# VITA-Group/UVC

Hardware: AMD Instinct MI355X
Metric: images/sec UVC Stage-1 step, DeiT-Tiny budget=0.5 (higher is better)
Workload: dtype bf16; 1 GPU; deit_tiny_patch16_224 Stage-1 UVC-train step, budget 0.5, per-GPU batch 512, 224x224x3 synthetic, soft distillation alpha 0.1, block gating on; global_batch=512, parallelism=dp1

## Files before the change

### include/uvc_kernels.h

```cpp
#ifndef UVC_KERNELS_H
#define UVC_KERNELS_H
#include <stdint.h>
#ifdef __cplusplus
extern "C" {
#endif

enum { UVC_F32 = 0, UVC_BF16 = 1 };

enum {
  UVC_EPI_NONE = 0,
  UVC_EPI_BIAS = 1,
  UVC_EPI_BIAS_GELU = 2,
  UVC_EPI_BIAS_RESID = 3,
  UVC_EPI_BIAS_RESID_GATE = 4,
  UVC_EPI_DGELU = 5,
  UVC_EPI_BIAS_GELU_OUT = 6,
  UVC_EPI_BIAS_GELU_GRAD = 7,
  UVC_EPI_MUL_AUX = 8,
  UVC_EPI_BIAS_GELU_GRAD_Q8 = 9,
  UVC_EPI_MUL_AUX_Q8 = 10
};
#define UVC_Q8_LO (-0.13f)
#define UVC_Q8_STEP (1.26f / 255.0f)

// ... 70 lines not shown

typedef struct uvc_attn_tok_args {
  const void* qkv;
  void* o;
  const void* dout;
  void* dqkv;
  int32_t B, N, H, head_dim, ntok, dtype;
  float scale;
  const int32_t* head_keep;
} uvc_attn_tok_args;
int uvc_attention_tok_fwd(const uvc_attn_tok_args* args, void* stream);
int uvc_attention_tok_bwd(const uvc_attn_tok_args* args, void* stream);

int uvc_copy_row_groups(const void* src, void* dst, int64_t groups, int64_t group_bytes, int64_t src_group_stride, int64_t dst_group_stride,
                        void* stream);

typedef struct uvc_ln_args {
  const void* x;
  const float* gamma; const float* beta;
  void* y; float* mean; float* rstd;
  const void* dy;
  void* dx;
  const void* add1; const float* a1;
  const void* add2; const float* a2;
  float* partial;
  float* dgamma; float* dbeta;
  float* dots;
  float eps, beta_acc;
  int32_t rows, D, rows_per_group, dtype, y_is_f32, dy_is_f32;
  int64_t group_stride;
// ... 102 lines not shown
```

### uvc_amd/_lib.py

```python
from __future__ import annotations

import ctypes as C
import os

import torch

_HERE = os.path.dirname(os.path.abspath(__file__))
LIB_PATH = os.path.join(_HERE, "libuvc_hip.so")


class UvcHipError(RuntimeError):
    pass


class uvc_dims(C.Structure):
    _fields_ = [("L", C.c_int32), ("H", C.c_int32), ("hd", C.c_int32), ("D", C.c_int32), ("F", C.c_int32)]


class uvc_hyper(C.Structure):
    _fields_ = [(n, C.c_float) for n in ("budget", "slr", "rlr", "glr", "ylr", "plr", "zlr", "sl2wd", "z_grad_clip",
                                         "gating_weight", "eps")] + \
               [(n, C.c_int32) for n in ("gating_interval", "use_gumbel", "enable_block_gating")]


# ... 146 lines not shown
    "uvc_resource": [C.POINTER(uvc_state), uvc_dims, uvc_hyper, VP, C.c_int32, VP, VP],
    "uvc_write_masks": [VP, VP, VP, uvc_dims, VP, VP, VP, VP, VP, VP],
    "uvc_gemm_nt": [C.POINTER(uvc_gemm_nt_args), VP],
    "uvc_gemm_nt_ln_supported": [I32, I32, I32, I32, I32],
    "uvc_gemm_nt_q8_supported": [I32, I32, I32, I32],
    "uvc_gemm_tn": [C.POINTER(uvc_gemm_tn_args), VP],
    "uvc_gemm_tn_workspace_bytes": [I32, I32, I32, C.POINTER(I64), C.POINTER(I32)],
    "uvc_attention_fwd": [C.POINTER(uvc_attn_args), VP],
    "uvc_attention_bwd": [C.POINTER(uvc_attn_args), VP],
    "uvc_attention_bwd_vdim": [C.POINTER(uvc_attn_args), VP],
    "uvc_qkv_attention_supported": [I32, I32, I32, I32, I32],
    "uvc_qkv_attention_fwd": [C.POINTER(uvc_qkv_attn_args), VP],
    "uvc_attention_tok_fwd": [C.POINTER(uvc_attn_tok_args), VP],
    "uvc_attention_tok_bwd": [C.POINTER(uvc_attn_tok_args), VP],
    "uvc_copy_row_groups": [VP, VP, I64, I64, I64, I64, VP],
    "uvc_layernorm_fwd": [C.POINTER(uvc_ln_args), VP],
    "uvc_layernorm_bwd": [C.POINTER(uvc_ln_args), VP],
    "uvc_layernorm_bwd_blocks": [I32],
    "uvc_layernorm_bwd_nblocks": [I32],
    "uvc_layernorm_bwd_reduce_batch": [C.POINTER(uvc_ln_reduce_item), I32, I32, F32, VP],
    "uvc_gemm_lnbwd_supported": [I32, I32, I32, I32],
    "uvc_gemm_lnbwd_nblocks": [I32],
    "uvc_gemm_nt_lnbwd": [C.POINTER(uvc_gemm_lnbwd_args), VP],
    "uvc_distill_loss": [C.POINTER(uvc_loss_args), VP],
    "uvc_grad_sqnorm": [VP, I64, VP, VP, I32, VP],
    "uvc_adamw_step": [C.POINTER(uvc_adamw_args), VP],
    "uvc_scale_by_clip": [VP, I64, VP, F32, VP],
    "uvc_patchify": [VP, VP, I32, I32, I32, I32, I32, VP],
    "uvc_assemble_tokens": [VP, VP, VP, VP, VP, VP, I32, I32, I32, I32, I32, VP],
    "uvc_assemble_tokens_bwd": [VP, VP, VP, VP, VP, VP, VP, VP, I32, I32, I32, I32, I32, I32, I32, F32, VP],
# ... 93 lines not shown
```

### uvc_amd/csrc/gemm.hip

```cpp
#include <type_traits>
#include "common.h"
#include "../../include/uvc_kernels.h"

template <typename T> struct Mma;
template <> struct Mma<bf16_t> {
  static constexpr int CH = 8;
  static constexpr int KSTEP = 32;
  typedef bf16x8 Frag;
  static __device__ __forceinline__ f32x4 mma(const Frag& a, const Frag& b, f32x4 c) {
    return __builtin_amdgcn_mfma_f32_16x16x32_bf16(a, b, c, 0, 0, 0);
  }
};
template <> struct Mma<float> {
  static constexpr int CH = 4;
  static constexpr int KSTEP = 16;
  typedef f32x4 Frag;
  static __device__ __forceinline__ f32x4 mma(const Frag& a, const Frag& b, f32x4 c) {
#pragma unroll
    for (int j = 0; j < 4; ++j) c = __builtin_amdgcn_mfma_f32_16x16x4f32(a[j], b[j], c, 0, 0, 0);
    return c;
  }
};

template <typename TS, typename T> struct ChunkLoad;
// ... 851 lines not shown
    E = En;
    if (next < ntiles) lstore(par ? sA0 : sA1);
    __syncthreads();
    par ^= 1;
  }
}

static bool wsn_ok(const NtArgs& a, int epi, bool a_f32) {
  return !a_f32 && a.N == 192 && (a.K == 768 || a.K == 576 || a.K == 512 || a.K == 256) && a.ldb == a.K && a.lda % 8 == 0 && a.ldc % 4 == 0 && a.ldr % 4 == 0 && a.M >= 4096 &&
         (epi == UVC_EPI_NONE || epi == UVC_EPI_BIAS || epi == UVC_EPI_BIAS_RESID || epi == UVC_EPI_BIAS_RESID_GATE);
}
template <int EPI, int KT, bool LN, int NST, bool RLOW> __global__ void k_gemm_wsn16_dma(NtArgs g);
template <int EPI, int KT, bool LN, int NST, bool RLOW>
static int launch_wsn16_dma(const NtArgs& a, hipStream_t st) {
  constexpr int NX_ = RLOW ? 7 : 13;
  constexpr int NA_ = (16 * (KT * 4 + 2) + 63) / 64, NI_ = NA_ + NX_ + (EPI == UVC_EPI_BIAS_RESID_GATE ? NX_ : 0);
  const int sh = NST * NI_ * 1024 + (LN ? 2 * 16 * 12 * 8 + 3 * 192 * 4 : 0);
  UVC_MAX_LDS(sh, k_gemm_wsn16_dma<EPI, KT, LN, NST, RLOW>);
  const int ntiles = ceil_div(a.M, 16);
  k_gemm_wsn16_dma<EPI, KT, LN, NST, RLOW><<<ntiles < 256 ? ntiles : 256, 768, sh, st>>>(a);
  UVC_CHECK_LAUNCH();
  return UVC_OK;
}
static bool wsn16_dma_ok(const NtArgs& a) {
  return a.M >= 16 && a.lda == a.K && a.ldr == 192 && a.ldc % 4 == 0 && (((uintptr_t)a.R | (uintptr_t)a.R2 | (uintptr_t)a.A) & 15) == 0;
}
template <typename TC, int KT>
static int launch_wsn16_kt(const NtArgs& a, int epi, hipStream_t st) {
  if constexpr (KT == 24 || KT == 16 || KT == 8) {
    constexpr bool RLOW = sizeof(TC) == 2;
    const bool ok = (!a.no_dma || a.ln_out) && wsn16_dma_ok(a) && (a.ln_out || a.M % 16 == 0);
// ... 50 lines not shown
    case 512: return launch_wsn_kt<TC, 16>(a, epi, st);
    default: return launch_wsn_kt<TC, 8>(a, epi, st);
  }
}

template <typename TA, typename T, typename TC>
static int launch_nt_epi(const NtArgs& a, int epi, hipStream_t st) {
  const int grid = ceil_div(ceil_div(a.M, NT_BM), 8) * 8 * ceil_div(a.N, NT_BN);
#define NT_CASE(E) case E: k_gemm_nt<TA, T, TC, E><<<grid, 256, 0, st>>>(a); break;
  switch (epi) {
    NT_CASE(UVC_EPI_NONE) NT_CASE(UVC_EPI_BIAS) NT_CASE(UVC_EPI_BIAS_GELU) NT_CASE(UVC_EPI_BIAS_RESID)
    NT_CASE(UVC_EPI_BIAS_RESID_GATE) NT_CASE(UVC_EPI_DGELU) NT_CASE(UVC_EPI_BIAS_GELU_OUT) NT_CASE(UVC_EPI_BIAS_GELU_GRAD) NT_CASE(UVC_EPI_MUL_AUX)
    default: return uvc_set_error_msg(UVC_ERR_ARG, "uvc_gemm_nt: unknown epilogue");
  }
#undef NT_CASE
  UVC_CHECK_LAUNCH();
  return UVC_OK;
}

int launch_nt256_f32(const NtArgs& a, int epi, hipStream_t st);
int launch_nt256_bf16(const NtArgs& a, int epi, hipStream_t st);
bool nt256_takes(const NtArgs& a, bool a_f32, bool any_size);
int launch_nt8p_f32(const NtArgs& a, int epi, int ri, hipStream_t st);
int launch_nt8p_bf16(const NtArgs& a, int epi, int ri, hipStream_t st);
bool nt8p_takes(const NtArgs& a, bool a_f32);
bool row384_fwd_ok(const NtArgs& a, int epi);
int launch_row384_fwd(const NtArgs& a, int epi, hipStream_t st);
static bool row384_fwd_fits(int64_t M, int64_t K) { return (M + 128) * K * 2 < (1ll << 31); }

extern "C" int uvc_gemm_nt_ln_supported(int32_t M, int32_t N, int32_t K, int32_t dtype, int32_t epilogue) {
// ... 49 lines not shown
      return uvc_set_error_msg(UVC_ERR_UNSUPPORTED, "uvc_gemm_nt: ln_out is not available for this problem (uvc_gemm_nt_ln_supported)");
    if (p->M % 16 != 0 && (p->C == (const void*)p->R || p->C == (const void*)p->R2))
      return uvc_set_error_msg(UVC_ERR_ARG, "uvc_gemm_nt: with ln_out and M % 16 != 0 the last row tile is computed twice: C must not alias R / R2");
    if (p->K == 192) return p->c_is_f32 ? launch_wsn16_dma<UVC_EPI_BIAS_RESID, 6, true, 7, false>(a, st) : launch_wsn16_dma<UVC_EPI_BIAS_RESID, 6, true, 7, true>(a, st);
    return p->c_is_f32 ? launch_wsn<float>(a, e, st) : launch_wsn<bf16_t>(a, e, st);
  }
  if (p->dtype == UVC_F32) {
    if (!p->a_is_f32 || !p->c_is_f32) return uvc_set_error_msg(UVC_ERR_ARG, "uvc_gemm_nt: float32 mode needs float32 A and C");
    return launch_nt_epi<float, float, float>(a, e, st);
  }
  if (p->dtype != UVC_BF16) return uvc_set_error_msg(UVC_ERR_ARG, "uvc_gemm_nt: dtype must be UVC_F32 or UVC_BF16");
  {
    if (!p->force_generic && !p->a_is_f32 && e == UVC_EPI_BIAS_RESID && p->K == 192 && p->N == 192 && a.ldb == 192 &&
        p->M >= 4096 && p->M % 16 == 0 && p->alpha == 1.0f && !p->alpha_ptr && wsn16_dma_ok(a))
      return p->c_is_f32 ? launch_wsn16_dma<UVC_EPI_BIAS_RESID, 6, false, 7, false>(a, st) : launch_wsn16_dma<UVC_EPI_BIAS_RESID, 6, false, 7, true>(a, st);
  }
  const bool ws = !generic && ws_ok(a, p->c_is_f32 ? 4 : 8);
  if (q8 && !ws) return uvc_set_error_msg(UVC_ERR_UNSUPPORTED, "uvc_gemm_nt: the one-byte GELU' epilogues exist in the K = 192 streaming kernel only");
  if (!generic && ws384_ok(a, e, p->c_is_f32 ? 4 : 8, p->a_is_f32 != 0)) {
    if (!p->c_is_f32 && a.N % 128 == 0 && a.N >= 512 && p->force_generic != 5) return launch_ws384<bf16_t, 8>(a, e, st);
    return p->c_is_f32 ? launch_ws384<float>(a, e, st) : launch_ws384<bf16_t>(a, e, st);
  }
  if (!generic && wsn_ok(a, e, p->a_is_f32 != 0))
    return p->c_is_f32 ? launch_wsn<float>(a, e, st) : launch_wsn<bf16_t>(a, e, st);
  if ((p->force_generic >> 8) == 1) {
    if (!nt8p_takes(a, p->a_is_f32 != 0)) return uvc_set_error_msg(UVC_ERR_UNSUPPORTED, "uvc_gemm_nt: shape not taken by the 8-phase kernel");
    return p->c_is_f32 ? launch_nt8p_f32(a, e, p->force_generic & 255, st) : launch_nt8p_bf16(a, e, p->force_generic & 255, st);
  }
  const bool few_tiles_wide = !p->c_is_f32 && a.N % 256 == 0 && nt8p_takes(a, p->a_is_f32 != 0);
  if (!generic && !a.no_dma && !(p->force_generic == 3 && few_tiles_wide && a.N < 1792) &&
      nt256_takes(a, p->a_is_f32 != 0, p->force_generic == 3 || p->force_generic == 4))
    return p->c_is_f32 ? launch_nt256_f32(a, e, st) : launch_nt256_bf16(a, e, st);
  if (!generic && !a.no_dma && few_tiles_wide && (a.M >= 2048 || p->force_generic == 3))
    return launch_nt8p_bf16(a, e, 0, st);
  if (p->a_is_f32) {
    if ((p->lda % 8) != 0) return uvc_set_error_msg(UVC_ERR_ARG, "uvc_gemm_nt: lda");
    if (ws) return p->c_is_f32 ? launch_ws<float, float>(a, e, st) : launch_ws<float, bf16_t>(a, e, st);
    return p->c_is_f32 ? launch_nt_epi<float, bf16_t, float>(a, e, st) : launch_nt_epi<float, bf16_t, bf16_t>(a, e, st);
  }
  if (ws) return p->c_is_f32 ? launch_ws<bf16_t, float>(a, e, st) : launch_ws<bf16_t, bf16_t>(a, e, st);
  return p->c_is_f32 ? launch_nt_epi<bf16_t, bf16_t, float>(a, e, st) : launch_nt_epi<bf16_t, bf16_t, bf16_t>(a, e, st);
}

template <typename T> struct Raw4L;
template <> struct Raw4L<float> {
  typedef f32x4 V;
  static __device__ __forceinline__ V ld(const float* p) { return *reinterpret_cast<const f32x4*>(p); }
  static __device__ __forceinline__ V zero() { return f32x4{0.f, 0.f, 0.f, 0.f}; }
  static __device__ __forceinline__ f32x4 cvt(const V& r) { return r; }
};
template <> struct Raw4L<bf16_t> {
  typedef u32x2 V;
  static __device__ __forceinline__ V ld(const bf16_t* p) { return *reinterpret_cast<const u32x2*>(p); }
  static __device__ __forceinline__ V zero() { return u32x2{0u, 0u}; }
// ... 377 lines not shown
    for (int q = 0; q < NWV; ++q) t += sRed[2 * q + tid];
    P[2 * D + tid] = t;
  }
}
#undef TIE4

template <int EPI, int KT, bool LN, int NST, bool RLOW>
__global__ __launch_bounds__(768) void k_gemm_wsn16_dma(NtArgs g) {
  typedef bf16_t T;
  typedef Mma<T> MM;
  constexpr int K = KT * 32, D = 192, NWV = 12;
  constexpr int ROWB = K * 2 + 32, SA = ROWB / 16;
  constexpr int NA = (16 * SA + 63) / 64;
  constexpr int RSZ = RLOW ? 2 : 4, RSL = D * RSZ / 16;
  constexpr int XS = RSL + 2, XB = XS * 16, NX = (16 * XS + 63) / 64;
  constexpr bool GATE = EPI == UVC_EPI_BIAS_RESID_GATE;
  constexpr int I_R = NA, I_R2 = I_R + NX, NI = I_R2 + (GATE ? NX : 0);
  constexpr int STAGE = NI * 1024;
  constexpr int NPW = (NI + NWV - 1) / NWV;
  constexpr int LN_BYTES = LN ? 2 * 16 * NWV * 8 + 3 * D * 4 : 0;
  static_assert(NST >= 3 && NPW <= 5 && NST * STAGE + LN_BYTES <= 160 * 1024, "ring does not fit");
  extern __shared__ __attribute__((aligned(16))) char smem[];
  const int tid = threadIdx.x, lane = tid & 63, gq = lane >> 4, li = lane & 15;
  const int w = __builtin_amdgcn_readfirstlane(tid >> 6);
  const T* __restrict__ W = reinterpret_cast<const T*>(g.B);
  char* __restrict__ C = reinterpret_cast<char*>(g.C);
  const int ntiles = (g.M + 15) / 16;
  const int n = w * 16 + gq * 4;
  float* const sRed = reinterpret_cast<float*>(smem + NST * STAGE);
  float* const sGB = sRed + 2 * 16 * NWV * 2;
  if (LN) {
    if (tid < D) { sGB[tid] = g.ln_gamma[tid]; sGB[D + tid] = g.ln_beta[tid]; sGB[2 * D + tid] = g.bias[tid]; }
  }
  const unsigned gaddr = lds_addr(sGB) + (unsigned)n * 4u;
  const unsigned redr = lds_addr(sRed) + (unsigned)(li * NWV * 8);
  typename MM::Frag bf[KT];
#pragma unroll
  for (int ks = 0; ks < KT; ++ks)
    bf[ks] = __builtin_bit_cast(typename MM::Frag, *reinterpret_cast<const u32x4*>(W + (size_t)(w * 16 + li) * K + (ks * 4 + gq) * 8));
  float alpha = g.alpha;
  if (g.alpha_ptr) alpha *= *g.alpha_ptr;
  float d0 = 0.f, d1 = 1.f;
  if (GATE) { d0 = g.dptr[0]; d1 = g.dptr[1]; }
  f32x4 bias4 = {0.f, 0.f, 0.f, 0.f};
  if (!LN) bias4 = *reinterpret_cast<const f32x4*>(g.bias + n);

  const char* rb[NPW]; unsigned rstride[NPW], rdst[NPW], loff[NPW];
#pragma unroll
  for (int q = 0; q < NPW; ++q) {
    int I = q * NWV + w;
    if (I >= NI) I = w;
    const int sl = (I - (I < I_R ? 0 : I < I_R2 ? I_R : I_R2)) * 64 + lane;
    rdst[q] = (unsigned)I * 1024u;
    if (I < I_R) {
      const int row = sl / SA, c = sl % SA;
      rb[q] = reinterpret_cast<const char*>(g.A); rstride[q] = K * 2u;
      loff[q] = row < 16 ? (unsigned)(row * K * 2 + (c < K / 8 ? c : 0) * 16) : 0u;
    } else {
      const int row = sl / XS, c = sl % XS;
      rb[q] = reinterpret_cast<const char*>(I < I_R2 ? g.R : g.R2); rstride[q] = (unsigned)(D * RSZ);
      loff[q] = row < 16 ? (unsigned)(row * D * RSZ + (c < RSL ? c : 0) * 16) : 0u;
    }
  }
  auto issue = [&](int tile, int st) {
    const int t = tile < ntiles ? tile : ntiles - 1;
    const unsigned r0 = (unsigned)min(t * 16, g.M - 16);
#pragma unroll
    for (int q = 0; q < NPW; ++q) {
      const char* src = rb[q] + ((unsigned long long)r0 * (unsigned long long)rstride[q] + (unsigned long long)loff[q]);
      char* dst = smem + st * STAGE + rdst[q];
      __builtin_amdgcn_global_load_lds((const void __attribute__((address_space(1)))*)src, (void __attribute__((address_space(3)))*)dst, 16, 0, 0);
    }
  };
  const unsigned s0 = lds_addr(smem);
  const unsigned fragoff = (unsigned)(li * ROWB + gq * 16), roff = (unsigned)(I_R * 1024 + li * XB + n * RSZ);

  int tile = blockIdx.x;
#pragma unroll
  for (int q = 0; q < NST - 1; ++q) issue(tile + q * gridDim.x, q);
// ... 64 lines not shown
    if (LN && have_prev) { ln_first(); ln_issue(std::integral_constant<int, 32>{}); }
    GROUP(1, fb, fa)
    if (LN && have_prev) { ln_acc(); ln_issue(std::integral_constant<int, 64>{}); }
    GROUP(2, fa, fb)
    if (LN && have_prev) {
      ln_acc();
      if constexpr (KT / 2 > 3) { lgr = ds_read128<0>(gaddr); lbr = ds_read128<D * 4>(gaddr); }
      else { lgr = ds_read128<0>(gaddr); lbr = ds_read128<D * 4>(gaddr); wait_lgkm<0>(); ln_finish(); }
    }
    GROUP(3, fb, fa)
    if (LN && have_prev && KT / 2 > 3) ln_finish();
    GROUP(4, fa, fb) GROUP(5, fb, fa)
    GROUP(6, fa, fb) GROUP(7, fb, fa) GROUP(8, fa, fb) GROUP(9, fb, fa) GROUP(10, fa, fb) GROUP(11, fb, fa)
#undef GROUP
#undef RD2
    typename Resid<typename std::conditional<RLOW, bf16_t, float>::type>::Raw4 rr, rr2;
    if constexpr (RLOW) {
      asm volatile("ds_read_b64 %0, %1" : "=v"(rr) : "v"(sb + roff));
      rr2 = rr;
      if (GATE) asm volatile("ds_read_b64 %0, %1 offset:%2" : "=v"(rr2) : "v"(sb + roff), "n"(NX * 1024));
    } else {
      rr = ds_read128<0>(sb + roff); rr2 = rr;
      if (GATE) rr2 = ds_read128<NX * 1024>(sb + roff);
    }
    typedef Resid<typename std::conditional<RLOW, bf16_t, float>::type> RS;
    if constexpr (!LN) {
      wait_vm<(NST - 2) * NPW>();
      wait_lgkm<0>();
      asm volatile("" : "+v"(rr), "+v"(rr2));
      __builtin_amdgcn_s_barrier();
      const f32x4 r = RS::f4(rr), r2 = RS::f4(rr2);
      float o[4];
#pragma unroll
      for (int e = 0; e < 4; ++e) {
        o[e] = epi_scale_bias(c0[e], alpha, bias4[e]);
        o[e] += r[e];
        if (GATE) o[e] = epi_gate_mix(o[e], r2[e], d0, d1);
      }
      char* cp = C + ((size_t)(min(tile * 16, g.M - 16) + li) * g.ldc + n) * RSZ;
      if constexpr (RLOW) { u32x2 q; q[0] = pack_bf16x2(o[0], o[1]); q[1] = pack_bf16x2(o[2], o[3]); *reinterpret_cast<u32x2*>(cp) = q; }
      else *reinterpret_cast<f32x4*>(cp) = f32x4{o[0], o[1], o[2], o[3]};
    } else {
      u32x4 bq = ds_read128<2 * D * 4>(gaddr);
      wait_lgkm<0>();
      asm volatile("" : "+v"(rr), "+v"(rr2), "+v"(bq));
      const f32x4 r = RS::f4(rr), r2 = RS::f4(rr2), bv = __builtin_bit_cast(f32x4, bq);
      float o[4];
#pragma unroll
      for (int e = 0; e < 4; ++e) {
        o[e] = epi_scale_bias(c0[e], alpha, bv[e]);
        o[e] += r[e];
// ... 1584 lines not shown
```

### uvc_amd/csrc/token_tail.hip

```cpp
#include "common.h"
#include "../../include/uvc_kernels.h"

namespace {

constexpr int HD = 64, NTH = 256, MAXN = 256, MAXT = 2;

template <typename T> struct Row;
template <> struct Row<bf16_t> {
  static constexpr int WORDS = 33;
  static __device__ __forceinline__ void put8(uint32_t* row, int c, const bf16_t* src) {
    const u32x4 v = *reinterpret_cast<const u32x4*>(src);
#pragma unroll
    for (int e = 0; e < 4; ++e) row[c * 4 + e] = v[e];
  }
  static __device__ __forceinline__ float get(const uint32_t* row, int d) {
    const uint32_t w = row[d >> 1];
    return __uint_as_float((d & 1) ? (w & 0xffff0000u) : (w << 16));
  }
  static __device__ __forceinline__ float dot(const uint32_t* row, const float* q) {
    float s = 0.f;
#pragma unroll 8
    for (int i = 0; i < 32; ++i) {
      const uint32_t w = row[i];
      s = __builtin_fmaf(__uint_as_float(w << 16), q[2 * i], s);
// ... 205 lines not shown
  const dim3 grid(p->H, p->B);
  if (bwd) k_attn_tok_bwd<T><<<grid, NTH, sh, st>>>(a);
  else k_attn_tok_fwd<T><<<grid, NTH, sh, st>>>(a);
  UVC_CHECK_LAUNCH();
  return UVC_OK;
}

__global__ __launch_bounds__(256) void k_copy_row_groups(const char* __restrict__ src, char* __restrict__ dst, int64_t pieces, int ppg,
                                                         int64_t sgs, int64_t dgs) {
  const int64_t i = (int64_t)blockIdx.x * 256 + threadIdx.x;
  if (i >= pieces) return;
  const int64_t gi = i / ppg, r = i % ppg;
  *reinterpret_cast<u32x4*>(dst + gi * dgs + r * 16) = *reinterpret_cast<const u32x4*>(src + gi * sgs + r * 16);
}

}

extern "C" int uvc_attention_tok_fwd(const uvc_attn_tok_args* p, void* stream) {
  if (int e = tok_check(p, false)) return e;
  return p->dtype == UVC_F32 ? tok_launch<float>(p, false, (hipStream_t)stream) : tok_launch<bf16_t>(p, false, (hipStream_t)stream);
}

extern "C" int uvc_attention_tok_bwd(const uvc_attn_tok_args* p, void* stream) {
  if (int e = tok_check(p, true)) return e;
  return p->dtype == UVC_F32 ? tok_launch<float>(p, true, (hipStream_t)stream) : tok_launch<bf16_t>(p, true, (hipStream_t)stream);
}

extern "C" int uvc_copy_row_groups(const void* src, void* dst, int64_t groups, int64_t group_bytes, int64_t src_group_stride, int64_t dst_group_stride,
                                   void* stream) {
  if (!src || !dst) return uvc_set_error_msg(UVC_ERR_ARG, "uvc_copy_row_groups: null pointer");
  if (groups <= 0 || group_bytes <= 0 || (group_bytes | src_group_stride | dst_group_stride) % 16 || (((uintptr_t)src | (uintptr_t)dst) & 15))
    return uvc_set_error_msg(UVC_ERR_ARG, "uvc_copy_row_groups: sizes, strides and pointers must be positive multiples of 16 bytes");
  const int64_t ppg = group_bytes / 16, pieces = groups * ppg;
  k_copy_row_groups<<<(unsigned)((pieces + 255) / 256), 256, 0, (hipStream_t)stream>>>((const char*)src, (char*)dst, pieces, (int)ppg, src_group_stride,
                                                                                      dst_group_stride);
  UVC_CHECK_LAUNCH();
  return UVC_OK;
}
```

### uvc_amd/csrc/vit_engine.hip

```cpp
#include "engine_host.h"

namespace {

int check_cfg(const uvc_vit_cfg* c) {
  if (!c) return uvc_set_error_msg(UVC_ERR_ARG, "uvc_vit: null cfg");
  if (c->depth <= 0 || c->depth > UVC_VIT_MAX_DEPTH) return uvc_set_error_msg(UVC_ERR_ARG, "uvc_vit: depth out of range");
  if (c->embed_dim != c->num_heads * 64) return uvc_set_error_msg(UVC_ERR_UNSUPPORTED, "uvc_vit: head_dim must be 64");
  if (c->embed_dim % 64 || c->hidden % 64 || c->embed_dim > 1024) return uvc_set_error_msg(UVC_ERR_UNSUPPORTED, "uvc_vit: embed_dim/hidden must be multiples of 64, embed_dim <= 1024");
  if (c->img_size % c->patch_size || c->patch_size % 4) return uvc_set_error_msg(UVC_ERR_ARG, "uvc_vit: img_size/patch_size");
  if (c->ntok != 1 && c->ntok != 2) return uvc_set_error_msg(UVC_ERR_ARG, "uvc_vit: ntok must be 1 or 2");
  if (c->dtype != UVC_F32 && c->dtype != UVC_BF16) return uvc_set_error_msg(UVC_ERR_ARG, "uvc_vit: dtype");
  if (c->num_classes <= 0 || c->num_classes % 8) return uvc_set_error_msg(UVC_ERR_UNSUPPORTED, "uvc_vit: num_classes must be a positive multiple of 8");
  const int np = (c->img_size / c->patch_size) * (c->img_size / c->patch_size);
  if (np > 1024) return uvc_set_error_msg(UVC_ERR_UNSUPPORTED, "uvc_vit: more than 1024 patches (the attention kernels take N <= 1026)");
  return UVC_OK;
}

struct BlockBufs {
  void* x; void* h1; void* qkv; void* o; float* lse; float* mean1; float* rstd1;
  void* x1; void* h2; float* mean2; float* rstd2; void* a; void* u;
};
struct TailBufs {
  void* xc; void* oc; void* x1c; void* h2c; float* mean2c; float* rstd2c; void* ac; void* uc; void* xoutc;
  void* gAc; void* dAc; void* dHc; void* gBc; void* dOc;
// ... 212 lines not shown
  memset(&a, 0, sizeof(a));
  if (layer >= 0 && c.io->head_keep && (bwd ? c.io->head_keep_bwd != 0 : !c.io->training)) a.head_keep = c.io->head_keep + (size_t)layer * c.d.H;
  a.qkv = b.qkv; a.o = c.w.tail.oc; a.dout = c.w.tail.dOc; a.dqkv = c.w.dqkv;
  a.B = c.d.B; a.N = c.d.N; a.H = c.d.H; a.head_dim = 64; a.ntok = c.d.ntok; a.dtype = c.d.dtype; a.scale = 0.125f;
  return bwd ? uvc_attention_tok_bwd(&a, c.st) : uvc_attention_tok_fwd(&a, c.st);
}
bool gp_q8(const Ctx& c, int rows, int Fe) {
  if (c.io->gelu_grad_bf16 || c.io->force_generic == 1) return false;
  if (c.io->fused_train_mlp && uvc_mlp_fused_supported(c.d.D, Fe, c.d.dtype)) return false;
  return uvc_gemm_nt_q8_supported(rows, Fe, c.d.D, c.d.dtype) != 0;
}
int gather_tok(const Ctx& c, const void* full, void* compact, size_t esz) {
  return uvc_copy_row_groups(full, compact, c.d.B, (int64_t)c.d.ntok * c.d.D * esz, (int64_t)c.d.N * c.d.D * esz, (int64_t)c.d.ntok * c.d.D * esz, c.st);
}
int scatter_tok(const Ctx& c, const void* compact, void* full, size_t esz) {
  return uvc_copy_row_groups(compact, full, c.d.B, (int64_t)c.d.ntok * c.d.D * esz, (int64_t)c.d.ntok * c.d.D * esz, (int64_t)c.d.N * c.d.D * esz, c.st);
}
int tail_block(const Ctx& c) {
  if (c.io->full_tail || c.d.N > 256 || c.d.ntok > 2) return -1;
  int last = -1;
  for (int l = 0; l < c.d.L; ++l)
    if (c.io->gate_d || !c.io->run_block || c.io->run_block[l] != 0) last = l;
  return last;
}

int setup(Ctx& c, const uvc_vit_cfg* cfg, const uvc_vit_io* io, void* stream, bool bwd) {
  TRY(check_cfg(cfg));
  if (!io || !io->params || !io->workspace || io->batch <= 0) return uvc_set_error_msg(UVC_ERR_ARG, "uvc_vit: null io member");
  if (cfg->dtype == UVC_BF16 && !io->shadow) return uvc_set_error_msg(UVC_ERR_ARG, "uvc_vit: bf16 mode needs the shadow buffer");
  if (!io->shadow) return uvc_set_error_msg(UVC_ERR_ARG, "uvc_vit: shadow buffer (W^T copies) missing");
  c.cfg = cfg; c.io = io; c.st = stream; c.d = dims_of(*cfg, io->batch);
// ... 255 lines not shown
    w.gAs[d.L] = w.gA_pp[0];
    for (int l = d.L - 1; l >= 0; --l) { if (runs(l)) ++cnt; w.gAs[l] = w.gA_pp[cnt & 1]; }
  }
  w.gA = w.gAs[d.L];
  int last_l = -1;
  for (int l = 0; l < d.L; ++l) { const int stage = d.L - l; if (stage >= sb && stage < se && runs(l)) { last_l = l; break; } }
  if (sb == 0) {
  TRY(nt(c, io->d_logits, 1, sh(c, so.head_wt), w.dhc, 0, d.B, d.D, d.NC, UVC_EPI_NONE, nullptr, nullptr, nullptr, nullptr, nullptr, nullptr, nullptr, 0,
         d.ntok * d.D));
  TRY(tn(c, io->d_logits, 1, w.hc, G + o.head_w, G + o.head_b, d.B, d.NC, d.D, nullptr, 0, d.ntok * d.D));
  if (d.ntok == 2) {
    TRY(nt(c, io->d_logits_dist, 1, sh(c, so.headd_wt), (char*)w.dhc + (size_t)d.D * d.tsz, 0, d.B, d.D, d.NC, UVC_EPI_NONE, nullptr, nullptr, nullptr,
           nullptr, nullptr, nullptr, nullptr, 0, d.ntok * d.D));
    TRY(tn(c, io->d_logits_dist, 1, (const char*)w.hc + (size_t)d.D * d.tsz, G + o.headd_w, G + o.headd_b, d.B, d.NC, d.D, nullptr, 0, d.ntok * d.D));
  }
  hipError_t he = hipMemsetAsync(w.gA, 0, (size_t)d.M * d.D * d.tsz, hs);
  if (he != hipSuccess) return uvc_set_error(he, __FILE__, __LINE__);
  if (tl >= 0) {
    TRY(ln_bwd(c, w.dhc, t.xoutc, o.norm_w, o.norm_b, w.meanf, w.rstdf, t.gAc, nullptr, nullptr, nullptr, nullptr, w.dotsraw + 2 * d.L, rh, 1, d.D));
    TRY(scatter_tok(c, t.gAc, w.gA, d.tsz));
  } else
  TRY(ln_bwd(c, w.dhc, w.xL, o.norm_w, o.norm_b, w.meanf, w.rstdf, w.gA, nullptr, nullptr, nullptr, nullptr, w.dotsraw + 2 * d.L, rh, d.ntok,
             (int64_t)d.N * d.D));
  }
  for (int l = d.L - 1; l >= 0; --l) {
    const int stage = d.L - l;
    if (stage < sb || stage >= se) continue;
    if (!io->gate_d && io->run_block && !io->run_block[l]) continue;
    const BlockBufs& b = w.blk[l];
    const int64_t* q = o.blk[l];
    const float* g0 = io->gate_d ? io->gate_d + 2 * l : nullptr;
    const float* g1 = io->gate_d ? io->gate_d + 2 * l + 1 : nullptr;
    const bool tail = l == tl;
    const int rows = tail ? d.B * d.ntok : d.M;
    void* const gA_in = g_in(l);
    w.gA = w.gAs[l]; w.gB = w.gBs[l]; w.dA = w.dAs[l]; w.dqkv = w.dqkvs[l];
    void* gA = tail ? t.gAc : gA_in; void* gB = tail ? t.gBc : w.gB; void* dA = tail ? t.dAc : w.dA; void* dH = tail ? t.dHc : w.dH;
    const void* fa = tail ? t.ac : b.a; const void* fu = tail ? t.uc : b.u; const void* fh2 = tail ? t.h2c : b.h2;
// ... 15 lines not shown
      TRY(nt(c, dA, 0, mc->w1t, dH, 0, rows, d.D, Fe, UVC_EPI_NONE));
      TRY(tn(c, dA, 0, fh2, mc->dw1, mc->db1, rows, Fe, d.D, nullptr, 0, 0, true));
      TRY(flush_tn(c));
      TRY(uvc_mlp_scatter_grads(mc->dw1, mc->dw2, mc->db1, mc->inv, P + q[9], G + q[11], d.D, d.F, Fe, G + q[8], G + q[10], G + q[9], 0.f, d.dtype,
                                c.side ? c.side : c.st));
    }
    c.tn_inline = false;
    if (fuse2)
      TRY(dgrad_ln_bwd(c, w.dA, sh(c, so.blk_wt[l][2]), d.F, b.x1, q[6], q[7], b.mean2, b.rstd2, w.gB, gA_in, g1, nullptr, nullptr, nullptr));
    else
    TRY(ln_bwd(c, dH, fx1, q[6], q[7], fm2, fr2, gB, gA, g1, nullptr, nullptr, nullptr, rows, 1, d.D));
    TRY(nt(c, gB, gf, sh(c, so.blk_wt[l][1]), tail ? t.dOc : w.dH, 0, rows, d.D, d.D, UVC_EPI_NONE));
    TRY(tn(c, gB, gf, tail ? t.oc : b.o, G + q[4], G + q[5], rows, d.D, d.D));
    if (tail) {
      TRY(attn_tok(c, b, true, l));
      const hipError_t he = hipMemsetAsync(w.gB, 0, (size_t)d.M * d.D * d.tsz, hs);
      if (he != hipSuccess) return uvc_set_error(he, __FILE__, __LINE__);
      TRY(scatter_tok(c, t.gBc, w.gB, d.tsz));
    } else
    TRY(attn(c, b, true, l));
    const bool fuse1 = lnb_fused_ok(c, 3 * d.D);
    if (!fuse1) TRY(nt(c, w.dqkv, 0, sh(c, so.blk_wt[l][0]), w.dH, 0, d.M, d.D, 3 * d.D, UVC_EPI_NONE));
    TRY(tn(c, w.dqkv, 0, b.h1, G + q[2], d.qkv_bias ? G + q[3] : nullptr, d.M, 3 * d.D, d.D));
    if (fuse1)
      TRY(dgrad_ln_bwd(c, w.dqkv, sh(c, so.blk_wt[l][0]), 3 * d.D, b.x, q[0], q[1], b.mean1, b.rstd1, w.gA, w.gB, nullptr, io->gate_d ? gA_in : nullptr, g0,
                       w.dotsraw + 2 * l));
    else
    TRY(ln_bwd(c, w.dH, b.x, q[0], q[1], b.mean1, b.rstd1, w.gA, w.gB, nullptr, io->gate_d ? gA_in : nullptr, g0, w.dotsraw + 2 * l, d.M, 1, d.D));
    TRY(flush_tn(c));
  }
  w.gA = g_in(-1);
  if (sb <= d.L + 1 && se > d.L + 1) {
// ... 12 lines not shown
```

### uvc_amd/ops.py

```python
from __future__ import annotations

import ctypes as C
from typing import Optional

import torch

from . import _lib as L
from ._lib import (EPI_BIAS, EPI_BIAS_GELU, EPI_BIAS_GELU_GRAD, EPI_BIAS_GELU_GRAD_Q8, EPI_BIAS_GELU_OUT, EPI_BIAS_RESID, EPI_BIAS_RESID_GATE, EPI_DGELU,
                   EPI_MUL_AUX, EPI_MUL_AUX_Q8, EPI_NONE, Q8_LO, Q8_STEP, UVC_BF16, UVC_F32)

__all__ = ["EPI_NONE", "EPI_BIAS", "EPI_BIAS_GELU", "EPI_BIAS_RESID", "EPI_BIAS_RESID_GATE", "EPI_DGELU", "UVC_F32",
           "UVC_BF16"]


def tdtype(dtype: int) -> torch.dtype:
    return torch.float32 if dtype == UVC_F32 else torch.bfloat16


def _chk(*ts):
    for t in ts:
        if t is None:
            continue
        L.require_cuda(t)
        if not t.is_contiguous():
# ... 118 lines not shown
    L.check(L.lib().uvc_attention_tok_fwd(C.byref(a), L.cur_stream()), "uvc_attention_tok_fwd")


def attention_tok_bwd(qkv, o, dout, dqkv, B, N, H, ntok, dtype):
    a = _attn_tok_args(qkv, o, B, N, H, ntok, dtype, dout, dqkv)
    L.check(L.lib().uvc_attention_tok_bwd(C.byref(a), L.cur_stream()), "uvc_attention_tok_bwd")


def copy_row_groups(src, dst, groups, group_bytes, src_group_stride, dst_group_stride):
    _chk(src)
    _chk(dst)
    L.check(L.lib().uvc_copy_row_groups(L.ptr(src), L.ptr(dst), groups, group_bytes, src_group_stride, dst_group_stride, L.cur_stream()),
            "uvc_copy_row_groups")


def _ln_args(x, gamma, beta, rows, D, dtype, rows_per_group=1, group_stride=None, eps=1e-6):
    a = L.uvc_ln_args()
    a.x, a.gamma, a.beta = L.ptr(x), L.ptr(gamma), L.ptr(beta)
    a.rows, a.D, a.rows_per_group, a.dtype = rows, D, rows_per_group, dtype
    a.group_stride = group_stride if group_stride is not None else D * rows_per_group
    a.eps = eps
    a.x_lowp = int(not _is_f32(x))
    return a


def layernorm_fwd(x, gamma, beta, y, mean, rstd, rows, D, dtype, rows_per_group=1, group_stride=None, eps=1e-6):
    _chk(x, gamma, beta, y, mean, rstd)
    a = _ln_args(x, gamma, beta, rows, D, dtype, rows_per_group, group_stride, eps)
    a.y, a.mean, a.rstd, a.y_is_f32 = L.ptr(y), L.ptr(mean), L.ptr(rstd), _is_f32(y)
    L.check(L.lib().uvc_layernorm_fwd(C.byref(a), L.cur_stream()), "uvc_layernorm_fwd")
# ... 350 lines not shown
```

Measured before the change: 47250 images/sec.

## Fuse memset into token scatter, add small-M GEMM and streaming no-epilogue path

```diff
diff --git a/include/uvc_kernels.h b/include/uvc_kernels.h
--- a/include/uvc_kernels.h
+++ b/include/uvc_kernels.h
@@ -108,6 +108,8 @@
 
 int uvc_copy_row_groups(const void* src, void* dst, int64_t groups, int64_t group_bytes, int64_t src_group_stride, int64_t dst_group_stride,
                         void* stream);
+
+int uvc_scatter_row_groups_zero(const void* src, void* dst, int64_t groups, int64_t group_bytes, int64_t dst_group_stride, void* stream);
 
 typedef struct uvc_ln_args {
   const void* x;
diff --git a/uvc_amd/_lib.py b/uvc_amd/_lib.py
--- a/uvc_amd/_lib.py
+++ b/uvc_amd/_lib.py
@@ -184,6 +184,7 @@
     "uvc_attention_tok_fwd": [C.POINTER(uvc_attn_tok_args), VP],
     "uvc_attention_tok_bwd": [C.POINTER(uvc_attn_tok_args), VP],
     "uvc_copy_row_groups": [VP, VP, I64, I64, I64, I64, VP],
+    "uvc_scatter_row_groups_zero": [VP, VP, I64, I64, I64, VP],
     "uvc_layernorm_fwd": [C.POINTER(uvc_ln_args), VP],
     "uvc_layernorm_bwd": [C.POINTER(uvc_ln_args), VP],
     "uvc_layernorm_bwd_blocks": [I32],
diff --git a/uvc_amd/csrc/gemm.hip b/uvc_amd/csrc/gemm.hip
--- a/uvc_amd/csrc/gemm.hip
+++ b/uvc_amd/csrc/gemm.hip
@@ -889,7 +889,7 @@
 template <int EPI, int KT, bool LN, int NST, bool RLOW>
 static int launch_wsn16_dma(const NtArgs& a, hipStream_t st) {
   constexpr int NX_ = RLOW ? 7 : 13;
-  constexpr int NA_ = (16 * (KT * 4 + 2) + 63) / 64, NI_ = NA_ + NX_ + (EPI == UVC_EPI_BIAS_RESID_GATE ? NX_ : 0);
+  constexpr int NA_ = (16 * (KT * 4 + 2) + 63) / 64, NI_ = NA_ + (EPI == UVC_EPI_NONE ? 0 : NX_) + (EPI == UVC_EPI_BIAS_RESID_GATE ? NX_ : 0);
   const int sh = NST * NI_ * 1024 + (LN ? 2 * 16 * 12 * 8 + 3 * 192 * 4 : 0);
   UVC_MAX_LDS(sh, k_gemm_wsn16_dma<EPI, KT, LN, NST, RLOW>);
   const int ntiles = ceil_div(a.M, 16);
@@ -970,6 +970,80 @@
     default: return uvc_set_error_msg(UVC_ERR_ARG, "uvc_gemm_nt: unknown epilogue");
   }
 #undef NT_CASE
+  UVC_CHECK_LAUNCH();
+  return UVC_OK;
+}
+
+constexpr int R16_PF = 4;
+struct R16Tile { u32x4 a[2], b[4][2]; };
+template <typename TA, typename TC, int EPI>
+__global__ __launch_bounds__(64) void k_gemm_nt_rows16(NtArgs g) {
+  typedef bf16_t T;
+  typedef Mma<T> MM;
+  constexpr int BK = 64;
+  __shared__ __attribute__((aligned(16))) float stg[16 * EP_LD];
+  const TA* __restrict__ A = reinterpret_cast<const TA*>(g.A);
+  const T* __restrict__ B = reinterpret_cast<const T*>(g.B);
+  const int lane = threadIdx.x, li = lane & 15, gq = lane >> 4;
+  const int ntn = (g.N + 63) / 64;
+  const int m0 = (blockIdx.x / ntn) * 16, n0 = (blockIdx.x % ntn) * 64;
+  const int m = m0 + li;
+  auto gload = [&](R16Tile& t, int k0) {
+    const u32x4 z = {0u, 0u, 0u, 0u};
+#pragma unroll
+    for (int ks = 0; ks < 2; ++ks) {
+      const int kc = k0 + (ks * 4 + gq) * 8;
+      t.a[ks] = (m < g.M && kc < g.K) ? ChunkLoad<TA, T>::ld(A + (size_t)m * g.lda + kc) : z;
+#pragma unroll
+      for (int j = 0; j < 4; ++j) {
+        const int n = n0 + j * 16 + li;
+        t.b[j][ks] = (n < g.N && kc < g.K) ? ChunkLoad<T, T>::ld(B + (size_t)n * g.ldb + kc) : z;
+      }
+    }
+  };
+  f32x4 acc[4];
+#pragma unroll
+  for (int j = 0; j < 4; ++j) acc[j] = f32x4{0.f, 0.f, 0.f, 0.f};
+  const int nk = (g.K + BK - 1) / BK;
+  R16Tile t[R16_PF];
+#pragma unroll
+  for (int p = 0; p < R16_PF; ++p)
+    if (p < nk) gload(t[p], p * BK);
+  for (int kt = 0; kt < nk; kt += R16_PF) {
+#pragma unroll
+    for (int p = 0; p < R16_PF; ++p) {
+      if (kt + p < nk) {
+#pragma unroll
+        for (int ks = 0; ks < 2; ++ks)
+#pragma unroll
+          for (int j = 0; j < 4; ++j)
+            acc[j] = MM::mma(__builtin_bit_cast(typename MM::Frag, t[p].b[j][ks]), __builtin_bit_cast(typename MM::Frag, t[p].a[ks]), acc[j]);
+        if (kt + p + R16_PF < nk) gload(t[p], (kt + p + R16_PF) * BK);
+      }
+    }
+  }
+  float alpha = g.alpha;
+  if (g.alpha_ptr) alpha *= *g.alpha_ptr;
+  float d0 = 0.f, d1 = 1.f;
+  if (EPI == UVC_EPI_BIAS_RESID_GATE) { d0 = g.dptr[0]; d1 = g.dptr[1]; }
+  float bias_v[OutVec<TC>::VN];
+  nt_load_bias<TC, EPI>(g, lane, n0, bias_v);
+#pragma unroll
+  for (int j = 0; j < 4; ++j) *reinterpret_cast<f32x4*>(stg + li * EP_LD + j * 16 + gq * 4) = acc[j];
+  __syncthreads();
+  nt_epilogue_rows<T, TC, EPI, 16>(g, stg, lane, m0, n0, alpha, d0, d1, bias_v);
+}
+static bool nt_rows16_takes(const NtArgs& a) { return (int64_t)ceil_div(a.M, NT_BM) * ceil_div(a.N, NT_BN) < 128; }
+template <typename TA, typename TC>
+static int launch_nt_rows16(const NtArgs& a, int epi, hipStream_t st) {
+  const int grid = ceil_div(a.M, 16) * ceil_div(a.N, 64);
+#define R16_CASE(E) case E: k_gemm_nt_rows16<TA, TC, E><<<grid, 64, 0, st>>>(a); break;
+  switch (epi) {
+    R16_CASE(UVC_EPI_NONE) R16_CASE(UVC_EPI_BIAS) R16_CASE(UVC_EPI_BIAS_GELU) R16_CASE(UVC_EPI_BIAS_RESID)
+    R16_CASE(UVC_EPI_BIAS_RESID_GATE) R16_CASE(UVC_EPI_DGELU) R16_CASE(UVC_EPI_BIAS_GELU_OUT) R16_CASE(UVC_EPI_BIAS_GELU_GRAD) R16_CASE(UVC_EPI_MUL_AUX)
+    default: return uvc_set_error_msg(UVC_ERR_ARG, "uvc_gemm_nt: unknown epilogue");
+  }
+#undef R16_CASE
   UVC_CHECK_LAUNCH();
   return UVC_OK;
 }
@@ -1049,6 +1123,9 @@
     if (!p->force_generic && !p->a_is_f32 && e == UVC_EPI_BIAS_RESID && p->K == 192 && p->N == 192 && a.ldb == 192 &&
         p->M >= 4096 && p->M % 16 == 0 && p->alpha == 1.0f && !p->alpha_ptr && wsn16_dma_ok(a))
       return p->c_is_f32 ? launch_wsn16_dma<UVC_EPI_BIAS_RESID, 6, false, 7, false>(a, st) : launch_wsn16_dma<UVC_EPI_BIAS_RESID, 6, false, 7, true>(a, st);
+    if (!p->force_generic && !p->a_is_f32 && e == UVC_EPI_NONE && p->K == 192 && p->N == 192 && a.ldb == 192 && a.lda == 192 && a.ldc % 4 == 0 &&
+        p->M >= 4096 && p->M % 16 == 0 && p->alpha == 1.0f && !p->alpha_ptr && (((uintptr_t)a.A | (uintptr_t)a.C) & 15) == 0)
+      return p->c_is_f32 ? launch_wsn16_dma<UVC_EPI_NONE, 6, false, 16, false>(a, st) : launch_wsn16_dma<UVC_EPI_NONE, 6, false, 16, true>(a, st);
   }
   const bool ws = !generic && ws_ok(a, p->c_is_f32 ? 4 : 8);
   if (q8 && !ws) return uvc_set_error_msg(UVC_ERR_UNSUPPORTED, "uvc_gemm_nt: the one-byte GELU' epilogues exist in the K = 192 streaming kernel only");
@@ -1068,11 +1145,14 @@
     return p->c_is_f32 ? launch_nt256_f32(a, e, st) : launch_nt256_bf16(a, e, st);
   if (!generic && !a.no_dma && few_tiles_wide && (a.M >= 2048 || p->force_generic == 3))
     return launch_nt8p_bf16(a, e, 0, st);
+  const bool rows16 = !p->force_generic && !ws && nt_rows16_takes(a);
   if (p->a_is_f32) {
     if ((p->lda % 8) != 0) return uvc_set_error_msg(UVC_ERR_ARG, "uvc_gemm_nt: lda");
+    if (rows16) return p->c_is_f32 ? launch_nt_rows16<float, float>(a, e, st) : launch_nt_rows16<float, bf16_t>(a, e, st);
     if (ws) return p->c_is_f32 ? launch_ws<float, float>(a, e, st) : launch_ws<float, bf16_t>(a, e, st);
     return p->c_is_f32 ? launch_nt_epi<float, bf16_t, float>(a, e, st) : launch_nt_epi<float, bf16_t, bf16_t>(a, e, st);
   }
+  if (rows16) return p->c_is_f32 ? launch_nt_rows16<bf16_t, float>(a, e, st) : launch_nt_rows16<bf16_t, bf16_t>(a, e, st);
   if (ws) return p->c_is_f32 ? launch_ws<bf16_t, float>(a, e, st) : launch_ws<bf16_t, bf16_t>(a, e, st);
   return p->c_is_f32 ? launch_nt_epi<bf16_t, bf16_t, float>(a, e, st) : launch_nt_epi<bf16_t, bf16_t, bf16_t>(a, e, st);
 }
@@ -1480,10 +1560,12 @@
   constexpr int NA = (16 * SA + 63) / 64;
   constexpr int RSZ = RLOW ? 2 : 4, RSL = D * RSZ / 16;
   constexpr int XS = RSL + 2, XB = XS * 16, NX = (16 * XS + 63) / 64;
-  constexpr bool GATE = EPI == UVC_EPI_BIAS_RESID_GATE;
-  constexpr int I_R = NA, I_R2 = I_R + NX, NI = I_R2 + (GATE ? NX : 0);
+  constexpr bool GATE = EPI == UVC_EPI_BIAS_RESID_GATE, RES = EPI != UVC_EPI_NONE;
+  static_assert(RES || !LN, "LayerNorm output: residual epilogues only");
+  constexpr int I_R = NA, I_R2 = I_R + (RES ? NX : 0), NI = I_R2 + (GATE ? NX : 0);
   constexpr int STAGE = NI * 1024;
   constexpr int NPW = (NI + NWV - 1) / NWV;
+  constexpr bool SOME = NI < NWV;
   constexpr int LN_BYTES = LN ? 2 * 16 * NWV * 8 + 3 * D * 4 : 0;
   static_assert(NST >= 3 && NPW <= 5 && NST * STAGE + LN_BYTES <= 160 * 1024, "ring does not fit");
   extern __shared__ __attribute__((aligned(16))) char smem[];
@@ -1509,13 +1591,13 @@
   float d0 = 0.f, d1 = 1.f;
   if (GATE) { d0 = g.dptr[0]; d1 = g.dptr[1]; }
   f32x4 bias4 = {0.f, 0.f, 0.f, 0.f};
-  if (!LN) bias4 = *reinterpret_cast<const f32x4*>(g.bias + n);
+  if (!LN && RES) bias4 = *reinterpret_cast<const f32x4*>(g.bias + n);
 
   const char* rb[NPW]; unsigned rstride[NPW], rdst[NPW], loff[NPW];
 #pragma unroll
   for (int q = 0; q < NPW; ++q) {
     int I = q * NWV + w;
-    if (I >= NI) I = w;
+    if (I >= NI) I = SOME ? 0 : w;
     const int sl = (I - (I < I_R ? 0 : I < I_R2 ? I_R : I_R2)) * 64 + lane;
     rdst[q] = (unsigned)I * 1024u;
     if (I < I_R) {
@@ -1529,6 +1611,7 @@
     }
   }
   auto issue = [&](int tile, int st) {
+    if (SOME && w >= NI) return;
     const int t = tile < ntiles ? tile : ntiles - 1;
     const unsigned r0 = (unsigned)min(t * 16, g.M - 16);
 #pragma unroll
@@ -1623,8 +1706,9 @@
     GROUP(6, fa, fb) GROUP(7, fb, fa) GROUP(8, fa, fb) GROUP(9, fb, fa) GROUP(10, fa, fb) GROUP(11, fb, fa)
 #undef GROUP
 #undef RD2
-    typename Resid<typename std::conditional<RLOW, bf16_t, float>::type>::Raw4 rr, rr2;
-    if constexpr (RLOW) {
+    typename Resid<typename std::conditional<RLOW, bf16_t, float>::type>::Raw4 rr = {}, rr2 = {};
+    if constexpr (!RES) {
+    } else if constexpr (RLOW) {
       asm volatile("ds_read_b64 %0, %1" : "=v"(rr) : "v"(sb + roff));
       rr2 = rr;
       if (GATE) asm volatile("ds_read_b64 %0, %1 offset:%2" : "=v"(rr2) : "v"(sb + roff), "n"(NX * 1024));
@@ -1643,7 +1727,7 @@
 #pragma unroll
       for (int e = 0; e < 4; ++e) {
         o[e] = epi_scale_bias(c0[e], alpha, bias4[e]);
-        o[e] += r[e];
+        if (RES) o[e] += r[e];
         if (GATE) o[e] = epi_gate_mix(o[e], r2[e], d0, d1);
       }
       char* cp = C + ((size_t)(min(tile * 16, g.M - 16) + li) * g.ldc + n) * RSZ;
diff --git a/uvc_amd/csrc/token_tail.hip b/uvc_amd/csrc/token_tail.hip
--- a/uvc_amd/csrc/token_tail.hip
+++ b/uvc_amd/csrc/token_tail.hip
@@ -243,6 +243,15 @@
   *reinterpret_cast<u32x4*>(dst + gi * dgs + r * 16) = *reinterpret_cast<const u32x4*>(src + gi * sgs + r * 16);
 }
 
+__global__ __launch_bounds__(256) void k_scatter_row_groups_zero(const char* __restrict__ src, char* __restrict__ dst, int64_t pieces, int ppg, int64_t dpg) {
+  const int64_t i = (int64_t)blockIdx.x * 256 + threadIdx.x;
+  if (i >= pieces) return;
+  const int64_t gi = i / dpg, r = i % dpg;
+  u32x4 v = {0u, 0u, 0u, 0u};
+  if (r < ppg) v = *reinterpret_cast<const u32x4*>(src + (gi * ppg + r) * 16);
+  *reinterpret_cast<u32x4*>(dst + i * 16) = v;
+}
+
 }
 
 extern "C" int uvc_attention_tok_fwd(const uvc_attn_tok_args* p, void* stream) {
@@ -253,6 +262,16 @@
 extern "C" int uvc_attention_tok_bwd(const uvc_attn_tok_args* p, void* stream) {
   if (int e = tok_check(p, true)) return e;
   return p->dtype == UVC_F32 ? tok_launch<float>(p, true, (hipStream_t)stream) : tok_launch<bf16_t>(p, true, (hipStream_t)stream);
+}
+
+extern "C" int uvc_scatter_row_groups_zero(const void* src, void* dst, int64_t groups, int64_t group_bytes, int64_t dst_group_stride, void* stream) {
+  if (!src || !dst) return uvc_set_error_msg(UVC_ERR_ARG, "uvc_scatter_row_groups_zero: null pointer");
+  if (groups <= 0 || group_bytes <= 0 || group_bytes > dst_group_stride || (group_bytes | dst_group_stride) % 16 || (((uintptr_t)src | (uintptr_t)dst) & 15))
+    return uvc_set_error_msg(UVC_ERR_ARG, "uvc_scatter_row_groups_zero: sizes, the stride and pointers must be positive multiples of 16 bytes, group_bytes <= dst_group_stride");
+  const int64_t dpg = dst_group_stride / 16, pieces = groups * dpg;
+  k_scatter_row_groups_zero<<<(unsigned)((pieces + 255) / 256), 256, 0, (hipStream_t)stream>>>((const char*)src, (char*)dst, pieces, (int)(group_bytes / 16), dpg);
+  UVC_CHECK_LAUNCH();
+  return UVC_OK;
 }
 
 extern "C" int uvc_copy_row_groups(const void* src, void* dst, int64_t groups, int64_t group_bytes, int64_t src_group_stride, int64_t dst_group_stride,
diff --git a/uvc_amd/csrc/vit_engine.hip b/uvc_amd/csrc/vit_engine.hip
--- a/uvc_amd/csrc/vit_engine.hip
+++ b/uvc_amd/csrc/vit_engine.hip
@@ -250,7 +250,7 @@
   return uvc_copy_row_groups(full, compact, c.d.B, (int64_t)c.d.ntok * c.d.D * esz, (int64_t)c.d.N * c.d.D * esz, (int64_t)c.d.ntok * c.d.D * esz, c.st);
 }
 int scatter_tok(const Ctx& c, const void* compact, void* full, size_t esz) {
-  return uvc_copy_row_groups(compact, full, c.d.B, (int64_t)c.d.ntok * c.d.D * esz, (int64_t)c.d.ntok * c.d.D * esz, (int64_t)c.d.N * c.d.D * esz, c.st);
+  return uvc_scatter_row_groups_zero(compact, full, c.d.B, (int64_t)c.d.ntok * c.d.D * esz, (int64_t)c.d.N * c.d.D * esz, c.st);
 }
 int tail_block(const Ctx& c) {
   if (c.io->full_tail || c.d.N > 256 || c.d.ntok > 2) return -1;
@@ -536,14 +536,15 @@
            nullptr, nullptr, nullptr, nullptr, 0, d.ntok * d.D));
     TRY(tn(c, io->d_logits_dist, 1, (const char*)w.hc + (size_t)d.D * d.tsz, G + o.headd_w, G + o.headd_b, d.B, d.NC, d.D, nullptr, 0, d.ntok * d.D));
   }
-  hipError_t he = hipMemsetAsync(w.gA, 0, (size_t)d.M * d.D * d.tsz, hs);
-  if (he != hipSuccess) return uvc_set_error(he, __FILE__, __LINE__);
   if (tl >= 0) {
     TRY(ln_bwd(c, w.dhc, t.xoutc, o.norm_w, o.norm_b, w.meanf, w.rstdf, t.gAc, nullptr, nullptr, nullptr, nullptr, w.dotsraw + 2 * d.L, rh, 1, d.D));
     TRY(scatter_tok(c, t.gAc, w.gA, d.tsz));
-  } else
+  } else {
+  const hipError_t he = hipMemsetAsync(w.gA, 0, (size_t)d.M * d.D * d.tsz, hs);
+  if (he != hipSuccess) return uvc_set_error(he, __FILE__, __LINE__);
   TRY(ln_bwd(c, w.dhc, w.xL, o.norm_w, o.norm_b, w.meanf, w.rstdf, w.gA, nullptr, nullptr, nullptr, nullptr, w.dotsraw + 2 * d.L, rh, d.ntok,
              (int64_t)d.N * d.D));
+  }
   }
   for (int l = d.L - 1; l >= 0; --l) {
     const int stage = d.L - l;
@@ -589,8 +590,6 @@
     TRY(tn(c, gB, gf, tail ? t.oc : b.o, G + q[4], G + q[5], rows, d.D, d.D));
     if (tail) {
       TRY(attn_tok(c, b, true, l));
-      const hipError_t he = hipMemsetAsync(w.gB, 0, (size_t)d.M * d.D * d.tsz, hs);
-      if (he != hipSuccess) return uvc_set_error(he, __FILE__, __LINE__);
       TRY(scatter_tok(c, t.gBc, w.gB, d.tsz));
     } else
     TRY(attn(c, b, true, l));
diff --git a/uvc_amd/ops.py b/uvc_amd/ops.py
--- a/uvc_amd/ops.py
+++ b/uvc_amd/ops.py
@@ -156,6 +156,13 @@
             "uvc_copy_row_groups")
 
 
+def scatter_row_groups_zero(src, dst, groups, group_bytes, dst_group_stride):
+    _chk(src)
+    _chk(dst)
+    L.check(L.lib().uvc_scatter_row_groups_zero(L.ptr(src), L.ptr(dst), groups, group_bytes, dst_group_stride, L.cur_stream()),
+            "uvc_scatter_row_groups_zero")
+
+
 def _ln_args(x, gamma, beta, rows, D, dtype, rows_per_group=1, group_stride=None, eps=1e-6):
     a = L.uvc_ln_args()
     a.x, a.gamma, a.beta = L.ptr(x), L.ptr(gamma), L.ptr(beta)
```

Measured after the change: 47440 images/sec, median of 6. No clear change (+0.4%).
